# lidongyv/Explicit-Context-Mapping-for-Stereo-Matching

Hardware: AMD Instinct MI355X
Metric: stereo-pairs/sec (cmfsm train step fwd+bwd+Adam) (higher is better)
Workload: dtype f32; 1 GPU; SceneFlow 960x540 (padded to 576) D=192 batch=4/GPU fwd+bwd+Adam (train.py path); arch=cmfsm, global_batch=4, parallelism=dp1, cost_volume=collapsed into class-indexed 2-D convolutions, launch=eager

## Files before the change

explicit-context-mapping-for-stereo-matching_amd/csrc/conv3d_c1.hip:

```cpp
#include "common.h"
#include "bf16.h"
#include "fp32_conv_stage.h"
#include "partial_sum.h"
#include <cstdlib>

namespace {

typedef float f32x16 __attribute__((ext_vector_type(16)));

typedef float f32x2 __attribute__((ext_vector_type(2)));
constexpr int VT_W = 32, VT_H = 16, VT_D = 8;
constexpr int VH_W = VT_W + 2, VH_H = VT_H + 2, VH_D = VT_D + 2;
constexpr int VROW = 36;
constexpr int VPOS = VH_D * VH_H * VH_W;
constexpr int VSLOTS = (VPOS + 255) / 256;
constexpr int V_X_FLOATS = VH_D * VH_H * VROW * 2;
constexpr int V_W_FLOATS = 16 * 27 * 2;
constexpr int V_LDS_BYTES = (V_X_FLOATS + V_W_FLOATS + 2) * 4;
static_assert(2 * V_LDS_BYTES <= 160 * 1024, "two workgroups per CU");
__device__ __forceinline__ int v_slot(int dz, int hy, int wx) { return ((dz * VH_H + hy) * VROW + wx + 2 * ((hy >> 1) & 1)) * 2; }

template <bool GN, class T = float>
__global__ __launch_bounds__(256, 2) void conv3d_c1_fwd_v(const T* __restrict__ x, const float* __restrict__ w,
                                                          float* __restrict__ y, int Ci, int D, int H, int W, int tiles_d,
                                                          int tiles_h, int tiles_w, const float* __restrict__ mean_rstd,
                                                          const float* __restrict__ gamma, const float* __restrict__ beta) {
    extern __shared__ __attribute__((aligned(16))) float smem[];
    float* Xs = smem;
    float* Ws = smem + V_X_FLOATS;
    int bid = ecm_xcd_tile(blockIdx.x, gridDim.x);
    const int td = bid % tiles_d; bid /= tiles_d;
    const int tw = bid % tiles_w; bid /= tiles_w;
    const int th = bid % tiles_h;
    const int b = bid / tiles_h;
    const int w0 = tw * VT_W, h0 = th * VT_H, d0 = td * VT_D;
    const int tid = threadIdx.x;
    const int lw = tid & 7, lh = (tid >> 3) & 7, ld = tid >> 6;
    const size_t HW = (size_t)H * W, DHW = (size_t)D * HW;
    const int npairs = Ci >> 1;

    for (int i = tid; i < Ci * 27; i += 256) {
        const int c = i / 27, tap = i - c * 27;
        Ws[((c >> 1) * 27 + tap) * 2 + (c & 1)] = w[i];
    }
    unsigned goff[VSLOTS];
    int lslot[VSLOTS];
#pragma unroll
    for (int k = 0; k < VSLOTS; ++k) {
        const int p = tid + 256 * k;
        const int dz = p / (VH_H * VH_W), r = p - dz * (VH_H * VH_W), hy = r / VH_W, wx = r - hy * VH_W;
        const int gz = d0 - 1 + dz, gy = h0 - 1 + hy, gx = w0 - 1 + wx;
        const bool ok = p < VPOS && (unsigned)gz < (unsigned)D && (unsigned)gy < (unsigned)H && (unsigned)gx < (unsigned)W;
        goff[k] = ok ? (unsigned)(((size_t)gz * H + gy) * W + gx) * (unsigned)sizeof(T) : 0x80000000u;
        lslot[k] = p < VPOS ? v_slot(dz, hy, wx) * 4 : (V_X_FLOATS + V_W_FLOATS) * 4;
        asm volatile("" : "+v"(goff[k]), "+v"(lslot[k]));
    }
    const auto xr = __builtin_amdgcn_make_buffer_rsrc(const_cast<T*>(x) + (size_t)b * Ci * DHW, 0,
                                                      (unsigned)((size_t)Ci * DHW * sizeof(T)), 0x00020000);
    const unsigned cstride = (unsigned)(DHW * sizeof(T));
    f32x2 rr[VSLOTS];
    auto fetch = [&](int pair) {
        const unsigned s0 = (unsigned)(2 * pair) * cstride;
#pragma unroll
        for (int k = 0; k < VSLOTS; ++k) {
            if constexpr (sizeof(T) == 4) {
                rr[k].x = __builtin_bit_cast(float, __builtin_amdgcn_raw_buffer_load_b32(xr, goff[k], s0, 0));
                rr[k].y = __builtin_bit_cast(float, __builtin_amdgcn_raw_buffer_load_b32(xr, goff[k], s0 + cstride, 0));
            } else {
                rr[k].x = bf2f(__builtin_amdgcn_raw_buffer_load_b16(xr, goff[k], s0, 0));
                rr[k].y = bf2f(__builtin_amdgcn_raw_buffer_load_b16(xr, goff[k], s0 + cstride, 0));
            }
        }
    };
    fetch(0);
    f32x2 acc[2][2][4];
#pragma unroll
    for (int a = 0; a < 2; ++a)
#pragma unroll
        for (int c = 0; c < 2; ++c)
#pragma unroll
            for (int i = 0; i < 4; ++i) acc[a][c][i] = f32x2{0.f, 0.f};
    const char* win0 = reinterpret_cast<const char*>(Xs) + v_slot(2 * ld, 2 * lh, 4 * lw) * 4;
    const char* win2 = reinterpret_cast<const char*>(Xs) + v_slot(2 * ld, 2 * lh + 2, 4 * lw) * 4;
    char* xs_c = reinterpret_cast<char*>(Xs);
    for (int pair = 0; pair < npairs; ++pair) {
        if (pair > 0) __syncthreads();
        if (GN) {
            const int c0 = 2 * pair;
            const float m0 = mean_rstd[(b * 32 + c0) * 2], r0 = mean_rstd[(b * 32 + c0) * 2 + 1];
            const float m1 = mean_rstd[(b * 32 + c0 + 1) * 2], r1 = mean_rstd[(b * 32 + c0 + 1) * 2 + 1];
            float a0, s0, a1, s1;
            gn_affine(m0, r0, gamma[c0], beta[c0], a0, s0);
            gn_affine(m1, r1, gamma[c0 + 1], beta[c0 + 1], a1, s1);
#pragma unroll
            for (int k = 0; k < VSLOTS; ++k) {
                const bool in = goff[k] != 0x80000000u;
                rr[k].x = in ? fmaxf(__builtin_fmaf(rr[k].x, a0, s0), 0.f) : 0.f;
                rr[k].y = in ? fmaxf(__builtin_fmaf(rr[k].y, a1, s1), 0.f) : 0.f;
            }
        }
#pragma unroll
        for (int k = 0; k < VSLOTS; ++k) *reinterpret_cast<f32x2*>(xs_c + lslot[k]) = rr[k];
        __syncthreads();
        if (pair + 1 < npairs) fetch(pair + 1);
        f32x2 wv[27];
#pragma unroll
        for (int t = 0; t < 27; ++t) wv[t] = *reinterpret_cast<const f32x2*>(Ws + (pair * 27 + t) * 2);
#pragma unroll
        for (int dz = 0; dz < 4; ++dz)
#pragma unroll
            for (int hy = 0; hy < 4; ++hy) {
                f32x2 row[6];
                const float4* rp = reinterpret_cast<const float4*>((hy < 2 ? win0 : win2) + ((dz * VH_H + (hy & 1)) * VROW) * 8);
#pragma unroll
                for (int q = 0; q < 3; ++q) {
                    const float4 v = rp[q];
                    row[2 * q] = f32x2{v.x, v.y};
                    row[2 * q + 1] = f32x2{v.z, v.w};
                }
#pragma unroll
                for (int od = 0; od < 2; ++od) {
                    const int kd = dz - od;
                    if (kd < 0 || kd > 2) continue;
#pragma unroll
                    for (int oh = 0; oh < 2; ++oh) {
                        const int kh = hy - oh;
                        if (kh < 0 || kh > 2) continue;
#pragma unroll
                        for (int kw = 0; kw < 3; ++kw)
#pragma unroll
                            for (int i = 0; i < 4; ++i)
                                acc[od][oh][i] = __builtin_elementwise_fma(row[i + kw], wv[(kd * 3 + kh) * 3 + kw], acc[od][oh][i]);
                    }
                }
            }
    }
    float* yb = y + (size_t)b * DHW;
    const int ow = w0 + 4 * lw;
#pragma unroll
    for (int od = 0; od < 2; ++od)
#pragma unroll
        for (int oh = 0; oh < 2; ++oh) {
            const int z = d0 + 2 * ld + od, yy = h0 + 2 * lh + oh;
            if (z >= D || yy >= H || ow >= W) continue;
            float* dst = yb + ((size_t)z * H + yy) * W + ow;
            float o[4];
#pragma unroll
            for (int i = 0; i < 4; ++i) o[i] = acc[od][oh][i].x + acc[od][oh][i].y;
            if (ow + 3 < W && (((size_t)z * H + yy) * W + ow) % 4 == 0 && (reinterpret_cast<size_t>(yb) & 15) == 0)
                *reinterpret_cast<float4*>(dst) = make_float4(o[0], o[1], o[2], o[3]);
            else
#pragma unroll
                for (int i = 0; i < 4; ++i)
                    if (ow + i < W) dst[i] = o[i];
        }
}

constexpr int MTH = 6, MTW = 30;
constexpr int MIH = MTH + 2, MPOS = MIH * 32;
constexpr int MXS = MPOS + 32;
constexpr int M_LDS_BYTES = (32 * MXS + 27 * MPOS) * 4;
static_assert(MPOS == 256, "one window position per thread");

__global__ __launch_bounds__(256, 2) void conv3d_c1_fwd(const float* __restrict__ x, const float* __restrict__ w,
                                                        float* __restrict__ y, int Ci, int D, int H, int W, int zchunk,
                                                        int tiles_z, int tiles_h, int tiles_w) {
    extern __shared__ __attribute__((aligned(16))) float smem[];
    float* Xs = smem;
    float* Ts = smem + 32 * MXS;
    int bid = blockIdx.x;
    const int tw = bid % tiles_w; bid /= tiles_w;
    const int th = bid % tiles_h; bid /= tiles_h;
    const int tz = bid % tiles_z;
    const int b = bid / tiles_z;
    const int z0 = tz * zchunk, z1 = z0 + zchunk < D ? z0 + zchunk : D;
    const int oh0 = th * MTH, ow0 = tw * MTW;
    const int tid = threadIdx.x, lane = tid & 63, wave = tid >> 6, l31 = lane & 31, half = lane >> 5;
    const size_t HW = (size_t)H * W, DHW = (size_t)D * HW;

    float wa[16];
#pragma unroll
    for (int kk = 0; kk < 16; ++kk) {
        const int ci = 2 * kk + half;
        wa[kk] = (l31 < 27 && ci < Ci) ? w[(size_t)ci * 27 + l31] : 0.f;
    }
    const int prow = tid >> 5, pcol = tid & 31;
    const int gyy = oh0 - 1 + prow, gx = ow0 - 1 + pcol;
    const bool inplane = (unsigned)gyy < (unsigned)H && (unsigned)gx < (unsigned)W;
    const unsigned inoff = (unsigned)(gyy * W + gx) * 4u;
    const unsigned plane_bytes = (unsigned)DHW * 4u;
    const int nci = Ci < 32 ? Ci : 32;
    const auto xrs = __builtin_amdgcn_make_buffer_rsrc(const_cast<float*>(x + (size_t)b * Ci * DHW), 0,
                                                       (unsigned)nci * plane_bytes, 0x00020000);
    float xr[32];
    auto prefetch = [&](int z) {
        const bool ok = inplane && (unsigned)z < (unsigned)D;
        const unsigned off = ok ? (unsigned)z * (unsigned)HW * 4u + inoff : 0x80000000u;
#pragma unroll
        for (int cc = 0; cc < 32; ++cc)
            xr[cc] = __builtin_bit_cast(float, __builtin_amdgcn_raw_buffer_load_b32(xrs, off + (unsigned)cc * plane_bytes, 0, 0));
    };
    const bool owner = tid < MTH * MTW;
    const int ohy = tid / MTW, oxo = tid - ohy * MTW;
    const bool ovalid = owner && oh0 + ohy < H && ow0 + oxo < W;
    float* yp = y + (size_t)b * DHW + (size_t)(oh0 + ohy) * W + (ow0 + oxo);
    float r_prev = 0.f, r_cur = 0.f;

    prefetch(z0 - 1);
    for (int z = z0 - 1; z <= z1; ++z) {
        __syncthreads();
#pragma unroll
        for (int cc = 0; cc < 32; ++cc) Xs[cc * MXS + tid] = xr[cc];
        __syncthreads();
        if (z < z1) prefetch(z + 1);
        f32x16 acc[2];
#pragma unroll
        for (int r = 0; r < 2; ++r)
#pragma unroll
            for (int i = 0; i < 16; ++i) acc[r][i] = 0.f;
#pragma unroll
        for (int kk = 0; kk < 16; ++kk)
#pragma unroll
            for (int r = 0; r < 2; ++r) {
                const float bv = Xs[(kk * 2 + half) * MXS + (wave * 2 + r) * 32 + l31];
                acc[r] = __builtin_amdgcn_mfma_f32_32x32x2f32(wa[kk], bv, acc[r], 0, 0, 0);
            }
#pragma unroll
        for (int r = 0; r < 2; ++r)
#pragma unroll
            for (int i = 0; i < 16; ++i) {
                const int tap = mfma32_row(i, half);
                if (tap < 27) Ts[tap * MPOS + (wave * 2 + r) * 32 + l31] = acc[r][i];
            }
        __syncthreads();
        if (owner) {
            float s0 = 0.f, s1 = 0.f, s2 = 0.f;
#pragma unroll
            for (int t9 = 0; t9 < 9; ++t9) {
                const int kh = t9 / 3, kw = t9 % 3;
                const int o = (ohy + kh) * 32 + oxo + kw;
                s0 += Ts[(0 * 9 + t9) * MPOS + o];
                s1 += Ts[(1 * 9 + t9) * MPOS + o];
                s2 += Ts[(2 * 9 + t9) * MPOS + o];
            }
            const float done = r_prev + s2;
            if (ovalid && z - 1 >= z0 && z - 1 < z1) yp[(size_t)(z - 1) * HW] = done;
            r_prev = r_cur + s1;
            r_cur = s0;
        }
    }
}

constexpr int DTH = 8, DTW = 128;
constexpr int DGW = DTW + 4;

__global__ __launch_bounds__(256) void conv3d_c1_dgrad(const float* __restrict__ gy, const float* __restrict__ w,
                                                       float* __restrict__ gx, int Ci, int D, int H, int W, int tiles_h,
                                                       int tiles_w) {
    __shared__ float Gs[3 * (DTH + 2) * DGW];
    int bid = blockIdx.x;
    const int tw = bid % tiles_w; bid /= tiles_w;
    const int th = bid % tiles_h; bid /= tiles_h;
    const int d = bid % D;
    const int b = bid / D;
    const int h0 = th * DTH, w0 = tw * DTW;
    const size_t HW = (size_t)H * W, DHW = (size_t)D * HW;
    const float* gb = gy + (size_t)b * DHW;
    for (int e = threadIdx.x; e < 3 * (DTH + 2) * (DTW + 2); e += 256) {
        const int xx = e % (DTW + 2), r = e / (DTW + 2);
        const int hy = r % (DTH + 2), dz = r / (DTH + 2);
        const int gz = d - 1 + dz, gh = h0 - 1 + hy, gw = w0 - 1 + xx;
        float v = 0.f;
        if ((unsigned)gz < (unsigned)D && (unsigned)gh < (unsigned)H && (unsigned)gw < (unsigned)W)
            v = gb[(size_t)gz * HW + (size_t)gh * W + gw];
        Gs[(dz * (DTH + 2) + hy) * DGW + xx] = v;
    }
    __syncthreads();
    const int hy = threadIdx.x >> 5, x4 = (threadIdx.x & 31) * 4;
    const int oh = h0 + hy, ow = w0 + x4;
    if (oh >= H || ow >= W) return;
    float g[9][6];
#pragma unroll
    for (int j = 0; j < 9; ++j)
#pragma unroll
        for (int i = 0; i < 6; ++i) g[j][i] = Gs[((j / 3) * (DTH + 2) + hy + (j % 3)) * DGW + x4 + i];
    const bool full = ow + 3 < W && (W & 3) == 0;
    float* op = gx + (size_t)b * Ci * DHW + (size_t)d * HW + (size_t)oh * W + ow;
    for (int ci = 0; ci < Ci; ++ci) {
        const float* wc = w + (size_t)ci * 27;
        float a0 = 0.f, a1 = 0.f, a2 = 0.f, a3 = 0.f;
#pragma unroll
        for (int kd = 0; kd < 3; ++kd)
#pragma unroll
            for (int kh = 0; kh < 3; ++kh)
#pragma unroll
                for (int kw = 0; kw < 3; ++kw) {
                    const float wv = wc[kd * 9 + kh * 3 + kw];
                    const int j = (2 - kd) * 3 + (2 - kh), i0 = 2 - kw;
                    a0 = fmaf(wv, g[j][i0 + 0], a0);
                    a1 = fmaf(wv, g[j][i0 + 1], a1);
                    a2 = fmaf(wv, g[j][i0 + 2], a2);
                    a3 = fmaf(wv, g[j][i0 + 3], a3);
                }
        float* o = op + (size_t)ci * DHW;
        if (full) ecm_st_stream(o, make_float4(a0, a1, a2, a3));
        else {
            o[0] = a0;
            if (ow + 1 < W) o[1] = a1;
            if (ow + 2 < W) o[2] = a2;
            if (ow + 3 < W) o[3] = a3;
        }
    }
}

constexpr int GTD = 2, GTH = 8, GTW = 32, GNV = GTD * GTH * GTW;
constexpr int GXSTR = GNV + 1;
constexpr int GRS = 35, GPS = 361;
constexpr int G_GYF = (GTD + 2) * GPS;
constexpr int G_LDS_BYTES = (32 * GXSTR + G_GYF) * 4;
static_assert((GTH + 2) * GRS <= GPS, "plane stride too small");

template <bool GN>
__global__ __launch_bounds__(256) void conv3d_c1_wgrad(const float* __restrict__ x, const float* __restrict__ gy,
                                                       float* __restrict__ partial, int B, int Ci, int D, int H, int W,
                                                       int tiles_d, int tiles_h, int tiles_w, const float* __restrict__ mean_rstd,
                                                       const float* __restrict__ gamma, const float* __restrict__ beta) {
    extern __shared__ __attribute__((aligned(16))) float smem[];
    float* Xs = smem;
    float* Gs = smem + 32 * GXSTR;
    float* Ps = Xs;
    const int tid = threadIdx.x, lane = tid & 63, wave = tid >> 6, l31 = lane & 31, half = lane >> 5;
    const size_t HW = (size_t)H * W, DHW = (size_t)D * HW;
    const int tap = l31 < 27 ? l31 : 0;
    const int kd = tap / 9, kh = (tap / 3) % 3, kw = tap % 3;
    const int toff = (2 - kd) * GPS + (2 - kh) * GRS + (2 - kw);
    f32x16 acc;
#pragma unroll
    for (int i = 0; i < 16; ++i) acc[i] = 0.f;
    const unsigned xplane = (unsigned)DHW * 4u;
    const int ntiles = B * tiles_d * tiles_h * tiles_w;
    constexpr int NGH = (GTD + 2) * (GTH + 2) * (GTW + 2);
    constexpr int PG = (NGH + 255) / 256;
    float xr[64], gr[PG];
    bool xin[2] = {false, false};
    int xb_next = 0;
    int gdst[PG];
#pragma unroll
    for (int j = 0; j < PG; ++j) {
        const int e = tid + j * 256;
        const int xx = e % (GTW + 2), hy = (e / (GTW + 2)) % (GTH + 2), dz = e / ((GTW + 2) * (GTH + 2));
        gdst[j] = e < NGH ? dz * GPS + hy * GRS + xx : -1;
    }
    const int nci = Ci < 32 ? Ci : 32;
    auto prefetch = [&](unsigned tile) {
        const bool live = tile < (unsigned)ntiles;
        unsigned r = live ? tile : 0u;
        const int tw = (int)(r % (unsigned)tiles_w); r /= (unsigned)tiles_w;
        const int th = (int)(r % (unsigned)tiles_h); r /= (unsigned)tiles_h;
        const int td = (int)(r % (unsigned)tiles_d);
        const int b = (int)(r / (unsigned)tiles_d);
        const int d0 = td * GTD, h0 = th * GTH, w0 = tw * GTW;
        unsigned off[2];
#pragma unroll
        for (int j = 0; j < 2; ++j) {
            const int v = tid + j * 256;
            const int xx = v % GTW, hy = (v / GTW) % GTH, dz = v / (GTW * GTH);
            const int gz = d0 + dz, gyy = h0 + hy, gx = w0 + xx;
            const bool ok = live && gz < D && gyy < H && gx < W;
            off[j] = ok ? (unsigned)(gz * (int)HW + gyy * W + gx) * 4u : 0x80000000u;
            if (GN) xin[j] = ok;
        }
        if (GN) xb_next = b;
        const auto xrs = __builtin_amdgcn_make_buffer_rsrc(const_cast<float*>(x + (size_t)b * Ci * DHW), 0,
                                                           (unsigned)nci * xplane, 0x00020000);
#pragma unroll
        for (int cc = 0; cc < 32; ++cc)
#pragma unroll
            for (int j = 0; j < 2; ++j)
                xr[cc * 2 + j] = __builtin_bit_cast(
                    float, __builtin_amdgcn_raw_buffer_load_b32(xrs, off[j] + (unsigned)cc * xplane, 0, 0));
        const auto grs = __builtin_amdgcn_make_buffer_rsrc(const_cast<float*>(gy + (size_t)b * DHW), 0, xplane, 0x00020000);
#pragma unroll
        for (int j = 0; j < PG; ++j) {
            const int e = tid + j * 256;
            const int xx = e % (GTW + 2), hy = (e / (GTW + 2)) % (GTH + 2), dz = e / ((GTW + 2) * (GTH + 2));
            const int gz = d0 - 1 + dz, gyy = h0 - 1 + hy, gx = w0 - 1 + xx;
            const bool ok = live && e < NGH && (unsigned)gz < (unsigned)D && (unsigned)gyy < (unsigned)H && (unsigned)gx < (unsigned)W;
            gr[j] = __builtin_bit_cast(float, __builtin_amdgcn_raw_buffer_load_b32(
                                                  grs, ok ? (unsigned)(gz * (int)HW + gyy * W + gx) * 4u : 0x80000000u, 0, 0));
        }
    };
    prefetch(blockIdx.x);
    for (unsigned tile = blockIdx.x; tile < (unsigned)ntiles; tile += gridDim.x) {
        __syncthreads();
        if (GN) {
#pragma unroll
            for (int cc = 0; cc < 32; ++cc) {
                const float m = mean_rstd[(xb_next * 32 + cc) * 2], r = mean_rstd[(xb_next * 32 + cc) * 2 + 1];
                float a, sh;
                gn_affine(m, r, gamma[cc], beta[cc], a, sh);
#pragma unroll
                for (int j = 0; j < 2; ++j) xr[cc * 2 + j] = xin[j] ? fmaxf(__builtin_fmaf(xr[cc * 2 + j], a, sh), 0.f) : 0.f;
            }
        }
#pragma unroll
        for (int cc = 0; cc < 32; ++cc)
#pragma unroll
            for (int j = 0; j < 2; ++j) Xs[cc * GXSTR + tid + j * 256] = xr[cc * 2 + j];
#pragma unroll
        for (int j = 0; j < PG; ++j)
            if (gdst[j] >= 0) Gs[gdst[j]] = gr[j];
        __syncthreads();
        prefetch(tile + gridDim.x);
        const float* xa = Xs + l31 * GXSTR + half;
        const float* gb = Gs + toff + half;
#pragma unroll
        for (int rr = 0; rr < GTD * GTH / 4; ++rr) {
            const int row = wave + rr * 4;
            const int dz = row / GTH, hy = row % GTH;
#pragma unroll
            for (int xx = 0; xx < GTW; xx += 2) {
                const float a = xa[(dz * GTH + hy) * GTW + xx];
                const float bv = l31 < 27 ? gb[dz * GPS + hy * GRS + xx] : 0.f;
                acc = __builtin_amdgcn_mfma_f32_32x32x2f32(a, bv, acc, 0, 0, 0);
            }
        }
    }
    __syncthreads();
#pragma unroll
    for (int i = 0; i < 16; ++i) {
        const int ci = mfma32_row(i, half);
        Ps[wave * 1024 + ci * 32 + l31] = acc[i];
    }
    __syncthreads();
    for (int e = tid; e < 1024; e += 256) {
        const int ci = e >> 5, t = e & 31;
        if (t < 27 && ci < Ci)
            partial[(size_t)blockIdx.x * Ci * 27 + ci * 27 + t] = (Ps[e] + Ps[1024 + e]) + (Ps[2048 + e] + Ps[3072 + e]);
    }
}

struct C1WgPlan { int tiles_d, tiles_h, tiles_w, P; long long ntiles, n; };
inline C1WgPlan c1_wgrad_plan(int B, int Ci, int D, int H, int W) {
    C1WgPlan p;
    p.tiles_d = (D + GTD - 1) / GTD; p.tiles_h = (H + GTH - 1) / GTH; p.tiles_w = (W + GTW - 1) / GTW;
    p.ntiles = (long long)B * p.tiles_d * p.tiles_h * p.tiles_w;
    p.P = (int)(p.ntiles < 512 ? p.ntiles : 512);
    p.n = (long long)Ci * 27;
    return p;
}

}

namespace {
template <bool GN, class T = float>
int launch_c1_fwd_v(const T* x, const float* w, float* y, int B, int Ci, int D, int H, int W, const float* mean_rstd,
                    const float* gamma, const float* beta, void* stream) {
    const int td = (D + VT_D - 1) / VT_D, th = (H + VT_H - 1) / VT_H, tw = (W + VT_W - 1) / VT_W;
    const long long nb = (long long)B * td * th * tw;
    if (nb > 0x7fffffffLL) return ECM_EUNSUP;
    const hipError_t e = ecm_allow_lds(reinterpret_cast<const void*>(conv3d_c1_fwd_v<GN, T>), V_LDS_BYTES);
    if (e != hipSuccess) return (int)e;
    hipLaunchKernelGGL((conv3d_c1_fwd_v<GN, T>), dim3((unsigned)nb), dim3(256), V_LDS_BYTES, ecm_stream(stream), x, w, y, Ci, D, H, W, td,
                       th, tw, mean_rstd, gamma, beta);
    return ECM_LAUNCH_RESULT();
}
}

extern "C" int ecm_conv3d_c1_gn_fwd(const float* x, const float* mean_rstd, const float* gamma, const float* beta, const float* w,
                                    float* y, int B, int Ci, int D, int H, int W, void* stream) {
    ECM_CHECK_ARG(x && mean_rstd && gamma && beta && w && y && B > 0 && Ci > 0 && D > 0 && H > 0 && W > 0);
    if (Ci != 32 || (long long)D * H * W * 4 * 32 >= 0x7fffffffLL) return ECM_EUNSUP;
    return launch_c1_fwd_v<true>(x, w, y, B, Ci, D, H, W, mean_rstd, gamma, beta, stream);
}

extern "C" int ecm_conv3d_c1_gn_fwd_bf16(const unsigned short* x, const float* mean_rstd, const float* gamma, const float* beta,
                                         const float* w, float* y, int B, int Ci, int D, int H, int W, void* stream) {
    ECM_CHECK_ARG(x && mean_rstd && gamma && beta && w && y && B > 0 && Ci > 0 && D > 0 && H > 0 && W > 0);
    if (Ci != 32 || (long long)D * H * W * 2 * 32 >= 0x7fffffffLL) return ECM_EUNSUP;
    return launch_c1_fwd_v<true, unsigned short>(x, w, y, B, Ci, D, H, W, mean_rstd, gamma, beta, stream);
}

extern "C" int ecm_conv3d_c1_fwd(const float* x, const float* w, float* y, int B, int Ci, int D, int H, int W, void* stream) {
    ECM_CHECK_ARG(x && w && y && B > 0 && Ci > 0 && D > 0 && H > 0 && W > 0);
    if (Ci > 32 || (long long)D * H * W * 4 * 32 >= 0x7fffffffLL) return ECM_EUNSUP;
    static const bool valu = [] { const char* v = getenv("ECM_C1_VALU"); return !(v && v[0] == '0'); }();
    if (valu && Ci % 2 == 0) return launch_c1_fwd_v<false>(x, w, y, B, Ci, D, H, W, nullptr, nullptr, nullptr, stream);
    const int tiles_h = (H + MTH - 1) / MTH, tiles_w = (W + MTW - 1) / MTW;
    const long long cols = (long long)B * tiles_h * tiles_w;
    int tiles_z = (int)((3 * 512 + cols - 1) / cols);
    if (tiles_z < 1) tiles_z = 1;
    if (tiles_z > (D + 7) / 8) tiles_z = (D + 7) / 8;
    const int zchunk = (D + tiles_z - 1) / tiles_z;
    tiles_z = (D + zchunk - 1) / zchunk;
    const long long nblk = cols * tiles_z;
    if (nblk > 0x7fffffffLL) return ECM_EUNSUP;
    {
        const hipError_t e = ecm_allow_lds(reinterpret_cast<const void*>(conv3d_c1_fwd), M_LDS_BYTES);
        if (e != hipSuccess) return (int)e;
    }
    hipLaunchKernelGGL(conv3d_c1_fwd, dim3((unsigned)nblk), dim3(256), M_LDS_BYTES, ecm_stream(stream), x, w, y, Ci, D, H, W,
                       zchunk, tiles_z, tiles_h, tiles_w);
    return ECM_LAUNCH_RESULT();
}

extern "C" int ecm_conv3d_c1_dgrad(const float* gy, const float* w, float* gx, int B, int Ci, int D, int H, int W, void* stream) {
    ECM_CHECK_ARG(gy && w && gx && B > 0 && Ci > 0 && D > 0 && H > 0 && W > 0);
    const int tiles_h = (H + DTH - 1) / DTH, tiles_w = (W + DTW - 1) / DTW;
    const long long nblk = (long long)B * D * tiles_h * tiles_w;
    if (nblk > 0x7fffffffLL) return ECM_EUNSUP;
    hipLaunchKernelGGL(conv3d_c1_dgrad, dim3((unsigned)nblk), dim3(256), 0, ecm_stream(stream), gy, w, gx, Ci, D, H, W, tiles_h,
                       tiles_w);
    return ECM_LAUNCH_RESULT();
}

extern "C" long long ecm_conv3d_c1_wgrad_scratch_bytes(int B, int Ci, int D, int H, int W) {
    if (B <= 0 || Ci <= 0 || D <= 0 || H <= 0 || W <= 0) return 0;
    const C1WgPlan p = c1_wgrad_plan(B, Ci, D, H, W);
    return p.P * p.n * (long long)sizeof(float);
}

namespace {
template <bool GN>
int launch_c1_wgrad(const float* x, const float* gy, float* gw, void* scratch, long long scratch_bytes, int B, int Ci, int D, int H,
                    int W, const float* mean_rstd, const float* gamma, const float* beta, void* stream) {
    const C1WgPlan p = c1_wgrad_plan(B, Ci, D, H, W);
    if (Ci > 32 || (long long)D * H * W * 4 * 32 >= 0x7fffffffLL || p.ntiles >= 0x7fffffffLL) return ECM_EUNSUP;
    if (scratch_bytes < p.P * p.n * (long long)sizeof(float)) return ECM_ESCRATCH;
    hipStream_t st = ecm_stream(stream);
    float* partial = static_cast<float*>(scratch);
    const int rc = stage_launch(conv3d_c1_wgrad<GN>, p.P, 1, 256, G_LDS_BYTES, (long long)D * H * W, st, x, gy, partial, B, Ci, D, H, W,
                                p.tiles_d, p.tiles_h, p.tiles_w, mean_rstd, gamma, beta);
    if (rc != 0) return rc;
    const int n = (int)p.n;
    hipLaunchKernelGGL(ecm_sum_partials<>, dim3((n + 31) / 32), dim3(256), 0, st, partial, gw, n, p.P);
    return ECM_LAUNCH_RESULT();
}
}

extern "C" int ecm_conv3d_c1_wgrad(const float* x, const float* gy, float* gw, void* scratch, long long scratch_bytes, int B,
                                   int Ci, int D, int H, int W, void* stream) {
    ECM_CHECK_ARG(x && gy && gw && scratch && B > 0 && Ci > 0 && D > 0 && H > 0 && W > 0);
    return launch_c1_wgrad<false>(x, gy, gw, scratch, scratch_bytes, B, Ci, D, H, W, nullptr, nullptr, nullptr, stream);
}

extern "C" int ecm_conv3d_c1_gn_wgrad(const float* x, const float* mean_rstd, const float* gamma, const float* beta, const float* gy,
                                      float* gw, void* scratch, long long scratch_bytes, int B, int Ci, int D, int H, int W,
                                      void* stream) {
    ECM_CHECK_ARG(x && mean_rstd && gamma && beta && gy && gw && scratch && B > 0 && Ci > 0 && D > 0 && H > 0 && W > 0);
    if (Ci != 32) return ECM_EUNSUP;
    return launch_c1_wgrad<true>(x, gy, gw, scratch, scratch_bytes, B, Ci, D, H, W, mean_rstd, gamma, beta, stream);
}
```

Before: 32.51 pairs/s.

## Stream depth planes through an LDS ring in the single-output-channel 3D conv forward

Restructures the Ci=32 to Co=1 3D conv forward so that each workgroup covers a taller tile (32 wide, 32 high, 16 deep) and walks the depth axis one halo plane at a time. Planes go through a three-slot LDS ring, and each thread keeps 16 depth accumulators in registers. The next plane's global loads are prefetched into registers while the current plane is being computed. The change cuts the halo re-read overhead and the LDS footprint, and reads weights straight from global memory instead of staging them in LDS. In exchange it adds one barrier per depth step, raises register pressure from the larger accumulator array, and launches fewer workgroups.

Result: no change. 32.50 pairs/s (-0.0%).

```diff
diff --git a/explicit-context-mapping-for-stereo-matching_amd/csrc/conv3d_c1.hip b/explicit-context-mapping-for-stereo-matching_amd/csrc/conv3d_c1.hip
--- a/explicit-context-mapping-for-stereo-matching_amd/csrc/conv3d_c1.hip
+++ b/explicit-context-mapping-for-stereo-matching_amd/csrc/conv3d_c1.hip
@@ -10,150 +10,156 @@
 
 typedef float f32x2 __attribute__((ext_vector_type(2)));
 constexpr int VT_W = 32, VT_H = 16, VT_D = 8;
-constexpr int VH_W = VT_W + 2, VH_H = VT_H + 2, VH_D = VT_D + 2;
-constexpr int VROW = 36;
-constexpr int VPOS = VH_D * VH_H * VH_W;
+constexpr int VM_H = 2, VM_D = 2;
+constexpr int VF_H = VM_H * VT_H, VF_D = VM_D * VT_D;
+constexpr int VH_W = VT_W + 2, VH_H = VF_H + 2;
+constexpr int VROW = 48;
+constexpr int VPOS = VH_H * VH_W;
 constexpr int VSLOTS = (VPOS + 255) / 256;
-constexpr int V_X_FLOATS = VH_D * VH_H * VROW * 2;
-constexpr int V_W_FLOATS = 16 * 27 * 2;
-constexpr int V_LDS_BYTES = (V_X_FLOATS + V_W_FLOATS + 2) * 4;
+constexpr int V_RING = 3;
+constexpr int V_STEPS = VF_D + 2;
+static_assert(V_STEPS % V_RING == 0, "a step's ring slot (s mod V_RING) must carry over from one channel pair to the next");
+constexpr int V_PLANE_FLOATS = VH_H * VROW * 2;
+constexpr int V_LDS_BYTES = (V_RING * V_PLANE_FLOATS + 2) * 4;
 static_assert(2 * V_LDS_BYTES <= 160 * 1024, "two workgroups per CU");
-__device__ __forceinline__ int v_slot(int dz, int hy, int wx) { return ((dz * VH_H + hy) * VROW + wx + 2 * ((hy >> 1) & 1)) * 2; }
 
 template <bool GN, class T = float>
 __global__ __launch_bounds__(256, 2) void conv3d_c1_fwd_v(const T* __restrict__ x, const float* __restrict__ w,
-                                                          float* __restrict__ y, int Ci, int D, int H, int W, int tiles_d,
+                                                          float* __restrict__ y, int Ci, int D, int H, int W, int tiles_z,
                                                           int tiles_h, int tiles_w, const float* __restrict__ mean_rstd,
                                                           const float* __restrict__ gamma, const float* __restrict__ beta) {
     extern __shared__ __attribute__((aligned(16))) float smem[];
-    float* Xs = smem;
-    float* Ws = smem + V_X_FLOATS;
     int bid = ecm_xcd_tile(blockIdx.x, gridDim.x);
-    const int td = bid % tiles_d; bid /= tiles_d;
+    const int tz = bid % tiles_z; bid /= tiles_z;
     const int tw = bid % tiles_w; bid /= tiles_w;
     const int th = bid % tiles_h;
     const int b = bid / tiles_h;
-    const int w0 = tw * VT_W, h0 = th * VT_H, d0 = td * VT_D;
+    const int w0 = tw * VT_W, h0 = th * VF_H, z0 = tz * VF_D;
+    const int nz = z0 + VF_D < D ? VF_D : D - z0;
     const int tid = threadIdx.x;
-    const int lw = tid & 7, lh = (tid >> 3) & 7, ld = tid >> 6;
+    const int lw = tid & 7, lh = tid >> 3;
     const size_t HW = (size_t)H * W, DHW = (size_t)D * HW;
     const int npairs = Ci >> 1;
 
-    for (int i = tid; i < Ci * 27; i += 256) {
-        const int c = i / 27, tap = i - c * 27;
-        Ws[((c >> 1) * 27 + tap) * 2 + (c & 1)] = w[i];
-    }
     unsigned goff[VSLOTS];
     int lslot[VSLOTS];
 #pragma unroll
     for (int k = 0; k < VSLOTS; ++k) {
         const int p = tid + 256 * k;
-        const int dz = p / (VH_H * VH_W), r = p - dz * (VH_H * VH_W), hy = r / VH_W, wx = r - hy * VH_W;
-        const int gz = d0 - 1 + dz, gy = h0 - 1 + hy, gx = w0 - 1 + wx;
-        const bool ok = p < VPOS && (unsigned)gz < (unsigned)D && (unsigned)gy < (unsigned)H && (unsigned)gx < (unsigned)W;
-        goff[k] = ok ? (unsigned)(((size_t)gz * H + gy) * W + gx) * (unsigned)sizeof(T) : 0x80000000u;
-        lslot[k] = p < VPOS ? v_slot(dz, hy, wx) * 4 : (V_X_FLOATS + V_W_FLOATS) * 4;
-        asm volatile("" : "+v"(goff[k]), "+v"(lslot[k]));
+        const int hy = p / VH_W, wx = p - hy * VH_W;
+        const int gy = h0 - 1 + hy, gx = w0 - 1 + wx;
+        const bool ok = p < VPOS && (unsigned)gy < (unsigned)H && (unsigned)gx < (unsigned)W;
+        goff[k] = ok ? (unsigned)((size_t)gy * W + gx) * (unsigned)sizeof(T) : 0x80000000u;
+        lslot[k] = p < VPOS ? (hy * VROW + wx) * 8 : V_RING * V_PLANE_FLOATS * 4;
     }
     const auto xr = __builtin_amdgcn_make_buffer_rsrc(const_cast<T*>(x) + (size_t)b * Ci * DHW, 0,
                                                       (unsigned)((size_t)Ci * DHW * sizeof(T)), 0x00020000);
-    const unsigned cstride = (unsigned)(DHW * sizeof(T));
-    f32x2 rr[VSLOTS];
-    auto fetch = [&](int pair) {
-        const unsigned s0 = (unsigned)(2 * pair) * cstride;
+    const unsigned cstride = (unsigned)(DHW * sizeof(T)), pstride = (unsigned)(HW * sizeof(T));
+    auto live = [&](int s) { const int z = z0 - 1 + s; return z >= 0 && z < D && s <= nz + 1; };
+    f32x2 rr[V_RING][VSLOTS];
+    auto fetch = [&](int pair, int s, f32x2* r) {
+        const bool on = pair < npairs && live(s);
+        const unsigned s0 = on ? (unsigned)(2 * pair) * cstride + (unsigned)(z0 - 1 + s) * pstride : 0u;
+        const unsigned kill = on ? 0u : 0x80000000u;
 #pragma unroll
         for (int k = 0; k < VSLOTS; ++k) {
             if constexpr (sizeof(T) == 4) {
-                rr[k].x = __builtin_bit_cast(float, __builtin_amdgcn_raw_buffer_load_b32(xr, goff[k], s0, 0));
-                rr[k].y = __builtin_bit_cast(float, __builtin_amdgcn_raw_buffer_load_b32(xr, goff[k], s0 + cstride, 0));
+                r[k].x = __builtin_bit_cast(float, __builtin_amdgcn_raw_buffer_load_b32(xr, goff[k] | kill, s0, 0));
+                r[k].y = __builtin_bit_cast(float, __builtin_amdgcn_raw_buffer_load_b32(xr, goff[k] | kill, s0 + cstride, 0));
             } else {
-                rr[k].x = bf2f(__builtin_amdgcn_raw_buffer_load_b16(xr, goff[k], s0, 0));
-                rr[k].y = bf2f(__builtin_amdgcn_raw_buffer_load_b16(xr, goff[k], s0 + cstride, 0));
+                r[k].x = bf2f(__builtin_amdgcn_raw_buffer_load_b16(xr, goff[k] | kill, s0, 0));
+                r[k].y = bf2f(__builtin_amdgcn_raw_buffer_load_b16(xr, goff[k] | kill, s0 + cstride, 0));
             }
         }
     };
-    fetch(0);
-    f32x2 acc[2][2][4];
-#pragma unroll
-    for (int a = 0; a < 2; ++a)
-#pragma unroll
-        for (int c = 0; c < 2; ++c)
-#pragma unroll
-            for (int i = 0; i < 4; ++i) acc[a][c][i] = f32x2{0.f, 0.f};
-    const char* win0 = reinterpret_cast<const char*>(Xs) + v_slot(2 * ld, 2 * lh, 4 * lw) * 4;
-    const char* win2 = reinterpret_cast<const char*>(Xs) + v_slot(2 * ld, 2 * lh + 2, 4 * lw) * 4;
-    char* xs_c = reinterpret_cast<char*>(Xs);
+#pragma unroll
+    for (int s = 0; s < V_RING; ++s) fetch(0, s, rr[s]);
+    f32x2 acc[VF_D][4];
+#pragma unroll
+    for (int j = 0; j < VF_D; ++j)
+#pragma unroll
+        for (int i = 0; i < 4; ++i) acc[j][i] = f32x2{0.f, 0.f};
+    char* xs_c = reinterpret_cast<char*>(smem);
+    const char* win = xs_c + (lh * VROW + 4 * lw) * 8;
     for (int pair = 0; pair < npairs; ++pair) {
-        if (pair > 0) __syncthreads();
+        f32x2 wv[27];
+#pragma unroll
+        for (int t = 0; t < 27; ++t) wv[t] = f32x2{w[(2 * pair) * 27 + t], w[(2 * pair + 1) * 27 + t]};
+        float a0 = 0.f, s0 = 0.f, a1 = 0.f, s1 = 0.f;
         if (GN) {
             const int c0 = 2 * pair;
             const float m0 = mean_rstd[(b * 32 + c0) * 2], r0 = mean_rstd[(b * 32 + c0) * 2 + 1];
             const float m1 = mean_rstd[(b * 32 + c0 + 1) * 2], r1 = mean_rstd[(b * 32 + c0 + 1) * 2 + 1];
-            float a0, s0, a1, s1;
             gn_affine(m0, r0, gamma[c0], beta[c0], a0, s0);
             gn_affine(m1, r1, gamma[c0 + 1], beta[c0 + 1], a1, s1);
-#pragma unroll
-            for (int k = 0; k < VSLOTS; ++k) {
-                const bool in = goff[k] != 0x80000000u;
-                rr[k].x = in ? fmaxf(__builtin_fmaf(rr[k].x, a0, s0), 0.f) : 0.f;
-                rr[k].y = in ? fmaxf(__builtin_fmaf(rr[k].y, a1, s1), 0.f) : 0.f;
-            }
-        }
-#pragma unroll
-        for (int k = 0; k < VSLOTS; ++k) *reinterpret_cast<f32x2*>(xs_c + lslot[k]) = rr[k];
+        }
         __syncthreads();
-        if (pair + 1 < npairs) fetch(pair + 1);
-        f32x2 wv[27];
-#pragma unroll
-        for (int t = 0; t < 27; ++t) wv[t] = *reinterpret_cast<const f32x2*>(Ws + (pair * 27 + t) * 2);
-#pragma unroll
-        for (int dz = 0; dz < 4; ++dz)
-#pragma unroll
-            for (int hy = 0; hy < 4; ++hy) {
-                f32x2 row[6];
-                const float4* rp = reinterpret_cast<const float4*>((hy < 2 ? win0 : win2) + ((dz * VH_H + (hy & 1)) * VROW) * 8);
-#pragma unroll
-                for (int q = 0; q < 3; ++q) {
-                    const float4 v = rp[q];
-                    row[2 * q] = f32x2{v.x, v.y};
-                    row[2 * q + 1] = f32x2{v.z, v.w};
-                }
-#pragma unroll
-                for (int od = 0; od < 2; ++od) {
-                    const int kd = dz - od;
-                    if (kd < 0 || kd > 2) continue;
-#pragma unroll
-                    for (int oh = 0; oh < 2; ++oh) {
-                        const int kh = hy - oh;
-                        if (kh < 0 || kh > 2) continue;
-#pragma unroll
-                        for (int kw = 0; kw < 3; ++kw)
-#pragma unroll
-                            for (int i = 0; i < 4; ++i)
-                                acc[od][oh][i] = __builtin_elementwise_fma(row[i + kw], wv[(kd * 3 + kh) * 3 + kw], acc[od][oh][i]);
+#pragma unroll
+        for (int s = 0; s < V_STEPS; ++s) {
+            f32x2* r = rr[s % V_RING];
+            char* slot = xs_c + (s % V_RING) * (V_PLANE_FLOATS * 4);
+            const bool lv = live(s);
+            if (lv) {
+                if (GN) {
+#pragma unroll
+                    for (int k = 0; k < VSLOTS; ++k) {
+                        const bool in = goff[k] != 0x80000000u;
+                        r[k].x = in ? fmaxf(__builtin_fmaf(r[k].x, a0, s0), 0.f) : 0.f;
+                        r[k].y = in ? fmaxf(__builtin_fmaf(r[k].y, a1, s1), 0.f) : 0.f;
                     }
                 }
-            }
+#pragma unroll
+                for (int k = 0; k < VSLOTS; ++k) *reinterpret_cast<f32x2*>(slot + lslot[k]) = r[k];
+            }
+            {
+                const int s2 = s + V_RING < V_STEPS ? s + V_RING : s + V_RING - V_STEPS;
+                const int p2 = s + V_RING < V_STEPS ? pair : pair + 1;
+                fetch(p2, s2, r);
+            }
+            if (lv) {
+                __syncthreads();
+#pragma unroll
+                for (int kh = 0; kh < 3; ++kh) {
+                    f32x2 row[6];
+                    const float4* rp = reinterpret_cast<const float4*>(win + (s % V_RING) * (V_PLANE_FLOATS * 4) + kh * (VROW * 8));
+#pragma unroll
+                    for (int q = 0; q < 3; ++q) {
+                        const float4 v = rp[q];
+                        row[2 * q] = f32x2{v.x, v.y};
+                        row[2 * q + 1] = f32x2{v.z, v.w};
+                    }
+#pragma unroll
+                    for (int kd = 0; kd < 3; ++kd) {
+                        const int j = s - kd;
+                        if (j < 0 || j >= VF_D) continue;
+#pragma unroll
+                        for (int kw = 0; kw < 3; ++kw)
+#pragma unroll
+                            for (int i = 0; i < 4; ++i)
+                                acc[j][i] = __builtin_elementwise_fma(row[i + kw], wv[(kd * 3 + kh) * 3 + kw], acc[j][i]);
+                    }
+                }
+            }
+        }
     }
     float* yb = y + (size_t)b * DHW;
-    const int ow = w0 + 4 * lw;
-#pragma unroll
-    for (int od = 0; od < 2; ++od)
-#pragma unroll
-        for (int oh = 0; oh < 2; ++oh) {
-            const int z = d0 + 2 * ld + od, yy = h0 + 2 * lh + oh;
-            if (z >= D || yy >= H || ow >= W) continue;
-            float* dst = yb + ((size_t)z * H + yy) * W + ow;
-            float o[4];
-#pragma unroll
-            for (int i = 0; i < 4; ++i) o[i] = acc[od][oh][i].x + acc[od][oh][i].y;
-            if (ow + 3 < W && (((size_t)z * H + yy) * W + ow) % 4 == 0 && (reinterpret_cast<size_t>(yb) & 15) == 0)
-                *reinterpret_cast<float4*>(dst) = make_float4(o[0], o[1], o[2], o[3]);
-            else
-#pragma unroll
-                for (int i = 0; i < 4; ++i)
-                    if (ow + i < W) dst[i] = o[i];
-        }
+    const int ow = w0 + 4 * lw, yy = h0 + lh;
+    if (yy >= H || ow >= W) return;
+#pragma unroll
+    for (int j = 0; j < VF_D; ++j) {
+        if (j >= nz) continue;
+        const int z = z0 + j;
+        float* dst = yb + ((size_t)z * H + yy) * W + ow;
+        float o[4];
+#pragma unroll
+        for (int i = 0; i < 4; ++i) o[i] = acc[j][i].x + acc[j][i].y;
+        if (ow + 3 < W && (((size_t)z * H + yy) * W + ow) % 4 == 0 && (reinterpret_cast<size_t>(yb) & 15) == 0)
+            *reinterpret_cast<float4*>(dst) = make_float4(o[0], o[1], o[2], o[3]);
+        else
+#pragma unroll
+            for (int i = 0; i < 4; ++i)
+                if (ow + i < W) dst[i] = o[i];
+    }
 }
 
 constexpr int MTH = 6, MTW = 30;
@@ -457,12 +463,13 @@
 int launch_c1_fwd_v(const T* x, const float* w, float* y, int B, int Ci, int D, int H, int W, const float* mean_rstd,
                     const float* gamma, const float* beta, void* stream) {
     const int td = (D + VT_D - 1) / VT_D, th = (H + VT_H - 1) / VT_H, tw = (W + VT_W - 1) / VT_W;
-    const long long nb = (long long)B * td * th * tw;
+    const int md = (td + VM_D - 1) / VM_D, mh = (th + VM_H - 1) / VM_H;
+    const long long nb = (long long)B * md * mh * tw;
     if (nb > 0x7fffffffLL) return ECM_EUNSUP;
     const hipError_t e = ecm_allow_lds(reinterpret_cast<const void*>(conv3d_c1_fwd_v<GN, T>), V_LDS_BYTES);
     if (e != hipSuccess) return (int)e;
-    hipLaunchKernelGGL((conv3d_c1_fwd_v<GN, T>), dim3((unsigned)nb), dim3(256), V_LDS_BYTES, ecm_stream(stream), x, w, y, Ci, D, H, W, td,
-                       th, tw, mean_rstd, gamma, beta);
+    hipLaunchKernelGGL((conv3d_c1_fwd_v<GN, T>), dim3((unsigned)nb), dim3(256), V_LDS_BYTES, ecm_stream(stream), x, w, y, Ci, D, H, W, md,
+                       mh, tw, mean_rstd, gamma, beta);
     return ECM_LAUNCH_RESULT();
 }
 }
```
